# W298/Surtr

Measured on AMD Instinct MI355X. Metric: fragments/sec, higher is better.
Workload: dtype f32

## Files before the change

surtr_amd/csrc/clip_core.h:

```cpp
#pragma once
#include <hip/hip_runtime.h>
#include <stdint.h>
#ifndef SURTR_LANES
#define SURTR_LANES 64
#define SURTR_LSH 6
#endif
#ifndef SURTR_WG
#define SURTR_WG 256
#endif
#if SURTR_LANES == 64
#define SURTR_WG_WIDE (4u * SURTR_WG)
#else
#define SURTR_WG_WIDE SURTR_WG
#endif
#define SURTR_NWAVE_WIDE (SURTR_WG_WIDE / SURTR_LANES)
#define SURTR_NWAVE (SURTR_WG / SURTR_LANES)
#ifndef SURTR_DBG
#define SURTR_DBG(...)
#endif

#ifdef SURTR_STAMP
__device__ unsigned long long g_stamp[96];
__device__ unsigned long long g_stamp2[64];
#ifdef SURTR_STAMP_SMALL
// ... 65 lines not shown
}

struct InLds
{
    typedef uint16_t off_t; typedef uint8_t len_t; typedef uint16_t idx_t;
    static constexpr uint32_t SENT = 0xFFFEu, REM = 0xFFFFu, MAXLEN = 255u;
};
struct InGlobal
{
    typedef uint32_t off_t; typedef uint32_t len_t; typedef uint32_t idx_t;
    static constexpr uint32_t SENT = 0xFFFFFFFEu, REM = 0xFFFFFFFFu, MAXLEN = 0x7FFFFFFFu;
};

template <class TT>
struct Topo
{
    typename TT::off_t* loff; typename TT::len_t* llen; typename TT::idx_t* ring;
    uint8_t* fc;
    int8_t* gcomp;
    float* pos;
    uint32_t* succ; uint32_t* pred; uint32_t* pcnt;
    uint32_t* aux0; uint32_t* aux1; uint32_t* aux2; uint32_t* aux3;
    uint2* blk;
    uint32_t capV, capH;
    uint32_t nS, nLive, hUsed;
    uint32_t kcur, n0cur; bool zmode;

    __device__ __forceinline__ int cmp(uint32_t v) const
    {
        if (zmode) return gcomp[v];
        const uint32_t f = fc[v];
        return f < kcur ? SURTR_DEAD : (f == kcur ? -1 : (v >= n0cur ? 2 : 1));
    }
    __device__ __forceinline__ bool alive(uint32_t v) const { return fc[v] >= kcur; }
    __device__ __forceinline__ void kill(uint32_t v) { fc[v] = (uint8_t)kcur; if (zmode) gcomp[v] = -1; }
};

struct Shared
{
    float4 planes[SURTR_MAXF + 1];
    union {
        float4 pmar[SURTR_MAXF + 1];
        uint32_t pw[4 * (SURTR_MAXF + 1)];
    };
    uint32_t hist[SURTR_MAXF + 1];
    uint32_t zhist[SURTR_MAXF + 1];
    uint32_t nzero[SURTR_MAXF + 1];
    uint32_t wsum[2 * SURTR_NWAVE_WIDE];
    uint32_t flagBad, flagErr;
    uint32_t deg7;
    uint32_t pf[3][8];
    uint32_t changed;
    uint32_t misc[8];
    uint32_t cutmask[4];
#ifdef SURTR_STAMP
    unsigned long long ph[16];
#endif
};

struct SolidIn
{
    const float* pos;
    const uint32_t* loff;
    const uint32_t* llen;
    const int32_t* nbr;
    uint32_t nv;
    const uint8_t* tri;
    const float* rad;
    const uint32_t* perm; const float4* posr_s; const float4* bsph;
};

__device__ __forceinline__ float plane_dist(const float4 pl, float x, float y, float z)
{
    float t = pl.x * x + pl.y * y;
    t = t + pl.z * z;
    return pl.w + t;
}

__device__ __forceinline__ int side_of(float s)
{
    if (fabsf(s) < 1.0e-10f) return 0;
    float m = -s;
    return m > 0.f ? 1 : (m < 0.f ? -1 : 0);
}

__device__ __forceinline__ uint32_t group_size() { return blockDim.x; }
__device__ __forceinline__ uint32_t group_waves() { return blockDim.x >> SURTR_LSH; }

__device__ __forceinline__ uint2 wave_incl_scan2(uint2 v)
{
    v.x += dpp_move<0x111, 0xF>(0u, v.x); v.y += dpp_move<0x111, 0xF>(0u, v.y);
    v.x += dpp_move<0x112, 0xF>(0u, v.x); v.y += dpp_move<0x112, 0xF>(0u, v.y);
    v.x += dpp_move<0x114, 0xF>(0u, v.x); v.y += dpp_move<0x114, 0xF>(0u, v.y);
    v.x += dpp_move<0x118, 0xF>(0u, v.x); v.y += dpp_move<0x118, 0xF>(0u, v.y);
    v.x += dpp_move<0x142, 0xA>(0u, v.x); v.y += dpp_move<0x142, 0xA>(0u, v.y);
    v.x += dpp_move<0x143, 0xC>(0u, v.x); v.y += dpp_move<0x143, 0xC>(0u, v.y);
    return v;
}

__device__ __forceinline__ uint2 wave_excl2(uint2 c)
{
    uint2 s = wave_incl_scan2(c);
    return make_uint2(s.x - c.x, s.y - c.y);
}

__device__ inline void scan_block_array(uint32_t nb, uint2* blk, Shared& sh, uint32_t& totC, uint32_t& totW)
{
    const uint32_t l = lane_id(), w = wave_id();
    uint2 carry = make_uint2(0u, 0u);
    for (uint32_t c0 = 0; c0 < nb; c0 += group_size())
    {
        const uint32_t i = c0 + threadIdx.x;
        uint2 x = make_uint2(0u, 0u);
        if (i < nb) x = blk[i];
        uint2 inc = wave_incl_scan2(x);
        if (l == SURTR_LANES - 1u) { sh.wsum[2 * w] = inc.x; sh.wsum[2 * w + 1] = inc.y; }
        __syncthreads();
        uint2 woff = make_uint2(0u, 0u), tot = make_uint2(0u, 0u);
        for (uint32_t q = 0; q < group_waves(); ++q)
        {
            const uint32_t a = sh.wsum[2 * q], bq = sh.wsum[2 * q + 1];
            if (q < w) { woff.x += a; woff.y += bq; }
            tot.x += a; tot.y += bq;
        }
        if (i < nb) blk[i] = make_uint2(carry.x + woff.x + inc.x - x.x, carry.y + woff.y + inc.y - x.y);
        carry.x += tot.x; carry.y += tot.y;
        __syncthreads();
    }
    totC = carry.x; totW = carry.y;
}

template <class Fn>
__device__ void scan_blocks(uint32_t n, uint2* blk, Shared& sh, Fn fn, uint32_t& totC, uint32_t& totW)
{
    const uint32_t nb = (n + SURTR_LANES - 1u) >> SURTR_LSH;
    const uint32_t l = lane_id(), w = wave_id();
    for (uint32_t b = w; b < nb; b += group_waves())
    {
        const uint32_t i = (b << SURTR_LSH) + l;
        uint2 c = make_uint2(0u, 0u);
        if (i < n) c = fn(i);
        uint2 s = wave_incl_scan2(c);
        if (l == SURTR_LANES - 1u) blk[b] = s;
    }
    __syncthreads();
    scan_block_array(nb, blk, sh, totC, totW);
}

template <class I>
__device__ __forceinline__ uint32_t face_next(const I* ring, uint32_t len, uint32_t prev)
{
    if (len <= 4u)
    {
        const uint32_t l1 = len > 1u ? 1u : 0u, l2 = len > 2u ? 2u : 0u, l3 = len > 3u ? 3u : 0u;
        const uint32_t e0 = ring[0], e1 = ring[l1], e2 = ring[l2], e3 = ring[l3];
        const uint32_t last = len == 4u ? e3 : (len == 3u ? e2 : (len == 2u ? e1 : e0));
        if (e0 == prev) return last;
        if (len > 1u && e1 == prev) return e0;
        if (len > 2u && e2 == prev) return e1;
        if (len > 3u && e3 == prev) return e2;
        return last;
    }
    uint32_t k = 0;
    while (k < len && (uint32_t)ring[k] != prev) ++k;
    if (k == 0) return (uint32_t)ring[len - 1];
    return (uint32_t)ring[k - 1];
// ... 766 lines not shown
        const uint32_t n0 = nS, n1 = nS + M;
        const uint32_t nref = T.nLive + (k ? sh.hist[k - 1u] : dropTotal) + M;
        if ((clist.l || cutcnt.l) && T.hUsed + 3u * M + 8u > wtop)
        {
            for (uint32_t i = tid; i < nC; i += group_size()) { if (clist.l) T.aux3[i] = clist.l[i]; if (cutcnt.l) T.aux2[i] = cutcnt.l[i]; }
            __syncthreads();
            clist.l = nullptr; cutcnt.l = nullptr; wtop = T.capH;
        }
        const uint32_t wfloor = T.hUsed + 3u * M;
        const WArr<uint16_t> srcv = carve16(M, wfloor, T.succ);
        const WArr<uint8_t> srcj = carve8(M, wfloor, T.aux1);
        const WArr<uint16_t> wpred = carve16(M, wfloor, T.pred);
        const WArr<uint16_t> wsave = carve16(M, wfloor, T.aux0);
        {
            bool dup = false;
            uint32_t run = 0;
            for (uint32_t q = 0; q < w; ++q) run += sh.wsum[q];
            for (uint32_t b = cb0; b < cb1; ++b)
            {
                const uint32_t i = (b << SURTR_LSH) + l;
                uint2 c = make_uint2(0u, 0u);
                uint32_t km = 0;
                if (i < nC) { km = cutcnt.get(i); c.x = (km & 0x8000u) ? (km & 0x7FFFu) : (uint32_t)__builtin_popcount(km); }
                const uint2 s2 = wave_incl_scan2(c);
                const uint32_t base = run;
                run += lane_bcast(s2.x, SURTR_LANES - 1u);
                if (i < nC && c.x)
                {
                    const uint32_t v = clist.get(i);
                    uint32_t t = base + s2.x - c.x;
                    if (MULTIWAVE && !(km & 0x8000u))
                    {
                        if (c.x >= 2u)
                        {
                            const I* r2 = T.ring + T.loff[v];
                            for (uint32_t mm = km; mm; mm &= mm - 1u)
                            {
                                const uint32_t ja = (uint32_t)__builtin_ctz(mm), ua = r2[ja];
                                for (uint32_t lo = km & ((1u << ja) - 1u); lo; lo &= lo - 1u) if ((uint32_t)r2[__builtin_ctz(lo)] == ua) dup = true;
                            }
                        }
                        for (uint32_t mm = km; mm; mm &= mm - 1u) { srcv.set(t, v); srcj.set(t, (uint32_t)__builtin_ctz(mm)); ++t; }
                        continue;
                    }
                    const I* r = T.ring + T.loff[v];
                    const uint32_t deg = T.llen[v];
                    for (uint32_t j0 = 0; j0 < deg; j0 += 4)
                    {
                        uint32_t u[4]; int cu[4];
#pragma unroll
                        for (int q = 0; q < 4; ++q) u[q] = r[j0 + q < deg ? j0 + q : deg - 1u];
#pragma unroll
                        for (int q = 0; q < 4; ++q) cu[q] = T.cmp(u[q] < TT::SENT ? u[q] : 0u);
#pragma unroll
                        for (int q = 0; q < 4; ++q)
                        {
                            const uint32_t j = j0 + q;
                            if (j >= deg || u[q] >= TT::SENT || cu[q] <= 0) continue;
                            srcv.set(t, v); srcj.set(t, j); ++t;
                            for (uint32_t jj = 0; jj < j; ++jj) if ((uint32_t)r[jj] == u[q]) dup = true;
                        }
                    }
                }
            }
            if (dup) pf[3] = 1;
            __syncthreads();
            STAMP(9);
            const bool ordered = pf[3] != 0;
            for (uint32_t t = tid; t < M; t += group_size())
            {
                const uint32_t v = srcv.get(t), j = srcj.get(t), fresh = n0 + t;
                I* r = T.ring + T.loff[v];
                const uint32_t u = r[j];
                const float ax = T.pos[3 * v], ay = T.pos[3 * v + 1], az = T.pos[3 * v + 2];
                const float bx = T.pos[3 * u], by = T.pos[3 * u + 1], bz = T.pos[3 * u + 2];
                const float sa = plane_dist(pl, ax, ay, az);
                const float sb = plane_dist(pl, bx, by, bz);
                const float inv = 1.f / (sb - sa);
                T.pos[3 * fresh] = (ax * sb - bx * sa) * inv;
                T.pos[3 * fresh + 1] = (ay * sb - by * sa) * inv;
                T.pos[3 * fresh + 2] = (az * sb - bz * sa) * inv;
                {
                    const float nx = T.pos[3 * fresh], ny = T.pos[3 * fresh + 1], nz = T.pos[3 * fresh + 2];
                    uint32_t f = SURTR_NEVER;
                    for (uint32_t q = k + 1u; q < F; ++q)
                    {
                        const int cq = side_of(plane_dist(sh.planes[q], nx, ny, nz));
                        if (cq < 0) { f = q; break; }
                        if (cq == 0) atomicAdd(&sh.nzero[q], 1u);
                    }
                    T.fc[fresh] = (uint8_t)f;
                    if (T.zmode) T.gcomp[fresh] = 2;
                }
                const uint32_t lo = T.hUsed + 3u * t;
                T.loff[fresh] = (typename TT::off_t)lo; T.llen[fresh] = 2;
                T.ring[lo] = (I)v; T.ring[lo + 1] = (I)u; T.ring[lo + 2] = (I)TT::REM;
                wpred.set(t, 0u);
                if (!ordered)
                {
                    I* ru = T.ring + T.loff[u];
                    const uint32_t du = T.llen[u];
                    for (uint32_t q = 0; q < du; ++q) if ((uint32_t)ru[q] == v) { ru[q] = (I)fresh; break; }
                    r[j] = (I)fresh;
                }
            }
            STAMP(10);
            if (ordered) __syncthreads();
            if (ordered && tid == 0)
            {
                COUNT(39);
                for (uint32_t t = 0; t < M; ++t)
                {
                    const uint32_t v = srcv.get(t), fresh = n0 + t, u = T.ring[T.loff[fresh] + 1u];
                    I* ru = T.ring + T.loff[u];
                    const uint32_t du = T.llen[u];
                    for (uint32_t q = 0; q < du; ++q) if ((uint32_t)ru[q] == v) { ru[q] = (I)fresh; break; }
                    T.ring[T.loff[v] + srcj.get(t)] = (I)fresh;
                }
            }
        }
        uint32_t hend = T.hUsed + 3u * M;
        if (tid == 0) sh.misc[6] = 0;
        __syncthreads();
        STAMP(5);

        bool serial = anyZero;
        if (!serial)
        {
            bool bad = false, longw = false;
            const WArr<uint16_t> wsucc = srcv;
            auto finish = [&](uint32_t t, uint32_t X, uint32_t c) {
                if (c >= TT::SENT || c < n0 || c == X || T.cmp(c) != 2) { bad = true; wsucc.set(t, X); }
                else
                {
                    wsucc.set(t, c);
                    wpred.set(c - n0, X);
                }
            };
            for (uint32_t t = tid; t < M; t += group_size())
            {
                const uint32_t X = n0 + t;
                uint32_t prev = X, c = T.ring[T.loff[X]], steps = 0;
                bool clipped;
                while (true)
                {
                    const uint32_t cc = c < TT::SENT ? c : 0u;
                    const int cm = T.cmp(cc); const uint32_t lo = T.loff[cc], len = T.llen[cc];
                    clipped = c < TT::SENT && cm == -1;
                    if (!clipped || steps >= SURTR_WALK0) break;
                    const uint32_t hold = c;
                    c = face_next(T.ring + lo, len, prev);
                    prev = hold; ++steps;
                }
                if (clipped) { wsave.set(t, prev + 1u); wsucc.set(t, c); longw = true; continue; }
                wsave.set(t, 0u);
                finish(t, X, c);
            }
            if (longw) pf[7] = 1;
            if (bad) pf[4] = 1;
            __syncthreads();
            STAMP(12);
            COUNT(43);
            if (pf[7] != 0)
            {
                COUNT(40);
                const uint32_t jfloor = T.hUsed + 3u * M;
                const WArr<uint16_t> chain = carve16(nC, jfloor, T.aux2);
                const WArr<uint16_t> jump = carve16(n0, jfloor, T.pcnt);
                for (uint32_t i = tid; i < nC; i += group_size())
                {
                    const uint32_t v = clist.get(i);
                    if (T.llen[v] != 3u) continue;
                    const uint32_t p = T.ring[T.loff[v]];
// ... 269 lines not shown
```

surtr_amd/csrc/prep_sorted.h:

```cpp
#pragma once
#include "wave_clip.h"

#define PS_NEVER 0x7Fu
#ifndef SURTR_PS_NB
#define SURTR_PS_NB 896u
#endif
#ifndef SURTR_SPH_FAN
#define SURTR_SPH_FAN 8u
#endif

namespace surtr {

struct SortedRings
{
    const SRow* row_s; const uint32_t* iperm;
    const float4* bsph2; const float4* bsph3;
};

__device__ __forceinline__ uint32_t ps_sphere_fc(const Shared& sh, const uint32_t F, const float4 sp, const uint32_t k0, uint32_t& kstop)
{
    const float mag = fabsf(sp.x) + fabsf(sp.y) + fabsf(sp.z) + sp.w;
    for (uint32_t k = k0; k < F; ++k)
    {
        const float4 mk = sh.pmar[k];
// ... 59 lines not shown
        if (k < F)
        {
            const float4 pk = sh.planes[k];
            const float n1 = fabsf(pk.x) + fabsf(pk.y) + fabsf(pk.z);
            const float n2 = sqrtf(pk.x * pk.x + pk.y * pk.y + pk.z * pk.z) * 1.0001f;
            sh.pmar[k] = make_float4(n2 * 1.00101f, 1.0e-5f * fabsf(pk.w), 1.0e-5f * n1, 0.f);
        }
    }
    if (tid == 0) { sh.flagErr = 0; sh.flagBad = 0; sh.deg7 = 0; for (int q = 0; q < 7; ++q) sh.misc[q] = 0; }
    const uint32_t nbV = (V + SURTR_LANES - 1u) >> SURTR_LSH;
    for (uint32_t q = tid; q < UBW; q += G) ub[q] = 0u;
    __syncthreads();
    const uint32_t nsb = (V + SURTR_SB - 1u) / SURTR_SB;
    const uint32_t nb2 = (nsb + SURTR_SPH_FAN - 1u) / SURTR_SPH_FAN, nb3 = (nb2 + SURTR_SPH_FAN - 1u) / SURTR_SPH_FAN;
    uint32_t* list2 = (uint32_t*)lbuf;
    uint32_t* list3 = list2 + nb2 + 8u;
    auto verts_in = [&](uint32_t g0, uint32_t g1) -> uint32_t {
        const uint32_t a = g0 * SURTR_SB, b = g1 * SURTR_SB;
        return (b < V ? b : V) - (a < V ? a : V);
    };
    for (uint32_t s3 = tid; s3 < nb3; s3 += G)
    {
        uint32_t ks = 0;
        const uint32_t f = ps_sphere_fc(sh, F, sr.bsph3[s3], 0u, ks);
        const uint32_t g0 = s3 * SURTR_SPH_FAN * SURTR_SPH_FAN;
        if (f != 0xFFu) atomicAdd(&sh.hist[f], verts_in(g0, g0 + SURTR_SPH_FAN * SURTR_SPH_FAN));
        else list3[atomicAdd(&sh.misc[1], 1u)] = s3 | (ks << 16);
    }
    __syncthreads();
    const uint32_t nU3 = sh.misc[1];
    for (uint32_t t = tid; t < nU3 * SURTR_SPH_FAN; t += G)
    {
        const uint32_t e3 = list3[t / SURTR_SPH_FAN];
        const uint32_t s2 = (e3 & 0xFFFFu) * SURTR_SPH_FAN + t % SURTR_SPH_FAN;
        if (s2 >= nb2) continue;
        uint32_t ks = 0;
        const uint32_t f = ps_sphere_fc(sh, F, sr.bsph2[s2], e3 >> 16, ks);
        if (f != 0xFFu) atomicAdd(&sh.hist[f], verts_in(s2 * SURTR_SPH_FAN, s2 * SURTR_SPH_FAN + SURTR_SPH_FAN));
        else list2[atomicAdd(&sh.misc[2], 1u)] = s2 | (ks << 16);
    }
    __syncthreads();
    const uint32_t nU2 = sh.misc[2];
    for (uint32_t t = tid; t < nU2 * SURTR_SPH_FAN; t += G)
    {
        const uint32_t e2 = list2[t / SURTR_SPH_FAN];
        const uint32_t sb = (e2 & 0xFFFFu) * SURTR_SPH_FAN + t % SURTR_SPH_FAN;
        if (sb >= nsb) continue;
        uint32_t ks = 0;
        const uint32_t f = ps_sphere_fc(sh, F, in.bsph[sb], e2 >> 16, ks);
        if (f != 0xFFu) atomicAdd(&sh.hist[f], verts_in(sb, sb + 1u));
        else atomicOr(&ub[sb >> 5], 1u << (sb & 31u));
    }
    __syncthreads();
    {
        uint32_t carry = 0;
        for (uint32_t q0 = 0; q0 < UBW; q0 += G)
        {
            const uint32_t q = q0 + tid;
            const uint32_t c = q < UBW ? (uint32_t)__builtin_popcount(ub[q]) : 0u;
            const uint32_t inc = wave_incl_scan2(make_uint2(c, 0u)).x;
            if (l == SURTR_LANES - 1u) sh.wsum[w] = inc;
            __syncthreads();
            uint32_t woff = 0, tot = 0;
            for (uint32_t x = 0; x < nw; ++x) { const uint32_t a = sh.wsum[x]; if (x < w) woff += a; tot += a; }
            if (q < UBW)
            {
                uint32_t at = carry + woff + inc - c;
                pre[q] = at;
                for (uint32_t m = ub[q]; m; m &= m - 1u) und[at++] = (uint16_t)(32u * q + (uint32_t)__builtin_ctz(m));
            }
            carry += tot;
            __syncthreads();
        }
        if (tid == 0) sh.misc[4] = carry;
    }
    __syncthreads();
    const uint32_t nUnd = sh.misc[4];
#ifdef SURTR_STAMP
    if (tid == 0 && V > 10000u) { atomicAdd(&g_stamp[45], (unsigned long long)nUnd); atomicAdd(&g_stamp[46], (unsigned long long)nsb); }
#endif
    STAMP(44);
    constexpr uint32_t GPW = SURTR_LANES / SURTR_SB;
    const uint32_t nWork = (nUnd + GPW - 1u) / GPW;
    for (uint32_t wb = w; wb < nWork; wb += nw)
    {
        const uint32_t sub = wb * GPW + l / SURTR_SB;
        const bool okg = sub < nUnd;
        const uint32_t i = (okg ? (uint32_t)und[sub] : 0u) * SURTR_SB + (l % SURTR_SB);
        const bool valid = okg && i < V;
        const float4 pr = in.posr_s[valid ? i : 0u];
        const float mag = fabsf(pr.x) + fabsf(pr.y) + fabsf(pr.z);
        uint32_t f = PS_NEVER, z = 0u;
        bool done = !valid, clear = true;
        for (uint32_t k = 0; k < F; ++k)
        {
            if (__all(done)) break;
            const float4 mk = sh.pmar[k];
            const float s = plane_dist(sh.planes[k], pr.x, pr.y, pr.z);
            const bool cut = s >= 1.0e-10f, zz = fabsf(s) < 1.0e-10f, live = !done;
            const bool far = fabsf(s) > __builtin_fmaf(pr.w, mk.x, __builtin_fmaf(mk.z, mag, mk.y));
            clear = clear & (far | !live);
            z |= (live & zz) ? 0x80u : 0u;
            f = (live & cut) ? k : f;
            done = done | cut;
        }
        const uint32_t at = sub * SURTR_SB + (l % SURTR_SB);
        if (valid) { if (at < kCap) vfc[at] = (uint8_t)(f | z); else vfc_g[at] = (uint8_t)(f | z); }
        const bool never = valid && f == PS_NEVER;
        const bool drop = valid && !never && clear;
        const bool need = valid && !never && !clear;
        wave_hist_add(sh.hist, f, drop);
        ps_append16(needy, &sh.misc[3], need, i);
        if (__ballot(never))
        {
            const uint32_t v = never ? in.perm[i] : 0u;
            const uint32_t deg = never ? in.llen[v] : 0u;
            if (never && z) sh.misc[5] = 1u;
            ps_append(klist, &sh.misc[6], never, i | ((f | z) << 16) | ((deg < 255u ? deg : 255u) << 24));
        }
    }
    __syncthreads();
    STAMP(0);
    const uint32_t nNeedy = sh.misc[3];
#ifdef SURTR_STAMP
    if (tid == 0 && V > 10000u) atomicAdd(&g_stamp[47], (unsigned long long)nNeedy);
#endif
    for (uint32_t t0 = w << SURTR_LSH; t0 < nNeedy; t0 += G)
    {
        const uint32_t t = t0 + l;
        const bool valid = t < nNeedy;
        const uint32_t i = valid ? (uint32_t)needy[t] : 0u;
        const SRow row = sr.row_s[i];
        uint32_t byte;
        {
            const uint32_t g = i / SURTR_SB, word = ub[g >> 5], bit = g & 31u;
            const uint32_t at = (pre[g >> 5] + (uint32_t)__builtin_popcount(word & ((1u << bit) - 1u))) * SURTR_SB + i % SURTR_SB;
            byte = (valid && at < kCap) ? (uint32_t)vfc[valid ? at : 0u] : 0u;
            if (valid && at >= kCap) byte = vfc_g[at];
        }
        const uint32_t f = byte & 0x7Fu;
        const uint32_t hd = row.w[0] & 0xFFFFu;
        const uint32_t deg = valid ? (hd & 7u) : 0u, notri = (hd >> 7) & 1u, big = (hd >> 6) & 1u;
        uint32_t uq[7], on[7], fq[7];
#pragma unroll
        for (int q = 0; q < 7; ++q)
        {
            const uint32_t x = row.w[(q + 1) >> 1];
            const uint32_t u = (uint32_t)q < deg ? (((q + 1) & 1) ? (x >> 16) : (x & 0xFFFFu)) : 0u;
            const uint32_t g = u / SURTR_SB, word = ub[g >> 5], bit = g & 31u;
            on[q] = ((uint32_t)q < deg ? 1u : 0u) & ((word >> bit) & 1u);
            uq[q] = (pre[g >> 5] + (uint32_t)__builtin_popcount(word & ((1u << bit) - 1u))) * SURTR_SB + u % SURTR_SB;
        }
#pragma unroll
        for (int q = 0; q < 7; ++q) fq[q] = (on[q] && uq[q] < kCap) ? ((uint32_t)vfc[uq[q]] & 0x7Fu) : f;
#pragma unroll
        for (int q = 0; q < 7; ++q) if (on[q] && uq[q] >= kCap) fq[q] = (uint32_t)vfc_g[uq[q]] & 0x7Fu;
        bool differ = false;
#pragma unroll
        for (int q = 0; q < 7; ++q) differ = differ | (fq[q] != f);
        const bool walk = valid && (big != 0u || (notri != 0u && !differ));
        const bool keep = valid && differ && !walk, drop = valid && !differ && !walk;
        if (keep && (byte & 0x80u)) sh.misc[5] = 1u;
        ps_append(klist, &sh.misc[6], keep, i | (byte << 16) | (deg << 24));
        if (__ballot(walk))
        {
            const uint32_t v = walk ? in.perm[i] : 0u;
            ps_append(walks, &sh.misc[0], walk, v | (f << 24));
        }
        wave_hist_add(sh.hist, f, drop);
        if (drop && (byte & 0x80u))
        {
            const float4 pr = in.posr_s[i];
            for (uint32_t k = 0; k < f; ++k)
                if (side_of(plane_dist(sh.planes[k], pr.x, pr.y, pr.z)) == 0) atomicAdd(&sh.zhist[k], 1u);
        }
    }
    __syncthreads();
    if (sh.misc[0] != 0u) prepass_exact<4>(in, F, sh, (unsigned long long*)nullptr, (uint2*)nullptr, walks, sh.misc[0], klist, &sh.misc[6], sr.iperm);
    __syncthreads();
    STAMP(1);
    const uint32_t n = sh.misc[6];
    for (uint32_t b = tid; b < nbV; b += G) { bmask[b] = 0ull; bblk[b] = make_uint2(0u, 0u); }
    __syncthreads();
    for (uint32_t t = tid; t < n; t += G)
    {
        const uint32_t ke = klist[t];
        const uint32_t v = in.perm[ke & 0xFFFFu], deg = ke >> 24;
        atomicOr(&bmask[v >> SURTR_LSH], 1ull << (v & (SURTR_LANES - 1u)));
// ... 222 lines not shown
```

surtr_amd/csrc/wave_clip.h:

```cpp
#pragma once
#include "clip_core.h"

#ifndef SURTR_WR
#define SURTR_WR 3584u
#endif
#ifndef SURTR_WNL
#define SURTR_WNL 2560u
#endif
#ifndef SURTR_WWALK0
#define SURTR_WWALK0 4u
#endif
#define WC_MAXF 64u
#define WC_MAXN 0x2000u
#define WC_BAIL 102
#define WC_SENT 0xFFFEu
#define WC_NONE 0xFFFFu
#define WC_WHY_WORDS 29u
static_assert(CUR_WC_WHY + WC_WHY_WORDS <= CUR_STATS_WORDS, "the why[] block ends inside what surtr_queue_stats copies out");
#define WC_RET(site) do { if (threadIdx.x == 0u) atomicAdd(&why[site], 1u); SURTR_DBG("record clip: pair handed on at site %d\n", site); return WC_BAIL; } while (0)
#ifdef SURTR_STAMP
__device__ unsigned long long g_wstamp[64];
__device__ unsigned long long g_wplane[32];
__device__ uint32_t g_wneed[4 * 8192];
#define WSTAMP_DECL unsigned long long ws_t0 = __builtin_readcyclecounter(), ws_t1
// ... 509 lines not shown
        auto fring = [&](uint32_t at) -> uint32_t { return at >= LT::kNL ? at - LT::kNL : at; };
        auto xof = [&](uint32_t t) -> uint32_t { return WC_MAXN + (t < fromf ? (uint32_t)W.freel[fring(fh0 + t)] : tbase + (t - fromf)); };
        for (uint32_t q = tid; q < bmw; q += G) wc_st32(B, bm + 2u * q, 0u);
        WSTAMP(3);
        WCOUNT(18, 1); WCOUNT(19, nC); WCOUNT(20, M); WCOUNT(21, nl);
#ifdef SURTR_STAMP
        if (tid == 0u) { const unsigned long long need = 2ull * (4u * rtop + (8u * LT::kNR - ltop)); if (need > W.ph[31]) W.ph[31] = need; if (k >= 2u && need > W.ph[29]) W.ph[29] = need; }
#endif
        auto kfn2 = [&](uint32_t i, uint32_t& aux) -> uint2 {
            const uint32_t id = clipped_id(i), km = wc_ld8(B, ckm8 + i);
            if (!(km & 0x80u)) { aux = id << 8; return make_uint2(0u, 0u); }
            aux = km | (id << 8) | (((tail_ld(id) >> 8) & 7u) << 24);
            return make_uint2(1u, (uint32_t)__builtin_popcount(km & 0x7Fu));
        };
        wc_rr_place<2>(W, sc, NI, st2, kfn2, [&](uint32_t i, uint32_t xc, uint32_t xm, uint2 c, uint32_t aux) {
            const uint32_t km = aux & 0x7Fu, id = (aux >> 8) & 0xFFFFu, len = aux >> 24;
            if (!c.x) { nout[i - xc] = (uint16_t)id; return; }
            wc_st16(B, cbase + i, xm);
            tail_st(id, 0x8000u | (len << 12) | i);
            if (i >= nCo) { W.freel[fring(fpush + (xc - nCo))] = (uint16_t)(id - WC_MAXN); wc_st16(B, clist + (xc - nCo), i); }
            uint32_t t = xm;
            for (uint32_t m = km; m; m &= m - 1u, ++t) { wc_st16(B, src + t, i | ((uint32_t)__builtin_ctz(m) << 12)); wc_st16(B, srcid + t, id); }
        });
        cur ^= 1u;
        WSTAMP(15);
        __syncthreads();
        WSTAMP(4);
        const uint32_t nref = nLive + (k ? SURTR_UNIFORM(W.hist[k - 1u]) : dropTotal) + M;
        bool fail = false;
        auto walk = [&](uint32_t& cv, uint32_t& pcv, uint32_t& p, WcRec& rc, uint32_t& steps, const uint32_t limit, const bool jump) -> uint32_t {
            while (true)
            {
                if (jump && p == 0u && pcv >= nCo)
                {
                    const uint32_t a = wc_ld32(B, nd + 2u * (pcv - nCo)), jx = a & 0xFFFFu;
                    if (jx != pcv) { pcv = jx; cv = clipped_id(jx); steps += a >> 16; rc = rec_of(cv); }
                }
                const uint32_t kmc = wc_ld8(B, ckm8 + pcv);
                if ((kmc >> p) & 1u) return wc_ld16(B, cbase + pcv) + (uint32_t)__builtin_popcount(kmc & ((1u << p) - 1u));
                if (steps >= limit) return WC_NONE;
                const uint32_t e = rc.e(p);
                if (((e >= WC_SENT ? 1u : 0u) | ((e < WC_MAXN ? 1u : 0u) & ((e < b0 ? 1u : 0u) | (e >= b1 ? 1u : 0u))) | (steps + 2u >= nref ? 1u : 0u)) != 0u)
                { SURTR_DBG("  wc walk: sentinel / not clipped / bound e=%u steps=%u nref=%u k=%u\n", e, steps, nref, k); fail = true; return WC_NONE; }
                ++steps;
                const WcRec re = rec_of(e);
                const uint32_t te = re.tail();
                if (!(te & 0x8000u)) { SURTR_DBG("  wc walk: vertex %u not clipped now (tail %x) k=%u\n", e, te, k); fail = true; return WC_NONE; }
                const uint32_t le = (te >> 12) & 7u, q = re.find(cv, le);
                if (q >= le) { SURTR_DBG("  wc walk: no way back k=%u\n", k); fail = true; return WC_NONE; }
                p = q ? q - 1u : le - 1u; cv = e; pcv = te & 0xFFFu; rc = re;
            }
        };
        auto arrive = [&](uint32_t t, uint32_t end) {
            wc_st16(B, wst + t, 0xFFFFu);
            uint32_t* word = (uint32_t*)(void*)(B + 2u * (size_t)(bm + 2u * (end >> 5)));
            const uint32_t before = atomicOr(word, 1u << (end & 31u));
            if (((end == t ? 1u : 0u) | ((before >> (end & 31u)) & 1u)) != 0u) { SURTR_DBG("  wc walk: ends on itself / second arrival t=%u end=%u k=%u\n", t, end, k); fail = true; }
            const uint32_t X = xof(t), Z = xof(end);
            wc_st16(B, 4u * (Z - WC_MAXN), X);
            wc_st16(B, 4u * (X - WC_MAXN) + 1u, Z);
        };
        bool paused = false;
        uint32_t myz0 = 0, myz1 = 0;
        uint16_t* nnow = W.nlist[cur];
        for (uint32_t t = tid; t < M; t += G)
        {
            const uint32_t s = wc_ld16(B, src + t);
            const uint32_t v = wc_ld16(B, srcid + t), j = s >> 12;
            uint32_t pcv = s & 0xFFFu, cv = v;
            WcRec rc = rec_of(cv);
            const uint32_t u = rc.e(j);
            const float4 pa = *(v < WC_MAXN ? g.gpos + v : g.cpos + (v - WC_MAXN));
            const float4 pb = *(u < WC_MAXN ? g.gpos + u : g.cpos + (u - WC_MAXN));
            WcW4 wru = WcW4{0u, 0u, 0u, 0u};
            if (u < WC_MAXN) wru = g.grec[u];
            const uint32_t lv = (rc.tail() >> 12) & 7u;
            uint32_t p = j ? j - 1u : lv - 1u, steps = 0;
            const uint32_t end = walk(cv, pcv, p, rc, steps, walk0, false);
            const uint32_t X = xof(t), ux = X - WC_MAXN;
            const float sa = plane_dist(pl, pa.x, pa.y, pa.z), sb = plane_dist(pl, pb.x, pb.y, pb.z);
            const float inv = 1.f / (sb - sa);
            const float nx = (pa.x * sb - pb.x * sa) * inv, ny = (pa.y * sb - pb.y * sa) * inv, nz = (pa.z * sb - pb.z * sa) * inv;
            g.cpos[ux] = make_float4(nx, ny, nz, 0.f);
            uint32_t f = SURTR_NEVER;
            for (uint32_t q = k + 1u; q < F; ++q)
            {
                const int cq = side_of(plane_dist(W.planes[q], nx, ny, nz));
                if (cq < 0) { f = q; break; }
                if (cq == 0) { if (q < 32u) myz0 |= 1u << q; else myz1 |= 1u << (q - 32u); }
            }
            wc_st32(B, 4u * ux + 2u, u | ((f | (3u << 8)) << 16));
            nnow[keepn + t] = (uint16_t)X;
            const WcRec ru = u < WC_MAXN ? WcRec{wru.a, wru.b, wru.c, wru.d} : wc_rec(B, 8u * (u - WC_MAXN), true);
            const uint32_t tu = ru.tail(), qu = ru.find(v, (tu >> 8) & 7u);
            if ((tu & 0x8000u) || qu >= ((tu >> 8) & 7u)) { SURTR_DBG("  wc patch: kept end does not link the clipped vertex k=%u\n", k); fail = true; }
            else if (u < WC_MAXN) { const uint16_t xv = (uint16_t)X; __builtin_memcpy(GB + 16u * (size_t)u + 2u * qu, &xv, 2); }
            else wc_st16(B, 4u * (u - WC_MAXN) + qu, X);
            if (end != WC_NONE) arrive(t, end);
            else { wc_st16(B, wst + t, pcv | (p << 12)); paused = true; }
        }
        const bool anyPaused = wc_any(W, ac, paused, 0u);
        WSTAMP(5);
        if (anyPaused)
        {
            WCOUNT(24, 1);
            for (uint32_t ci = tid; ci < nCn; ci += G)
            {
                const uint32_t i = wc_ld16(B, clist + ci);
                const uint32_t c = clipped_id(i);
                const WcRec r = rec_of(c);
                const uint32_t e0 = r.e(0u);
                uint32_t nx = i, d = 0;
                if (!(wc_ld8(B, ckm8 + i) & 1u) && e0 >= WC_MAXN && e0 < WC_SENT)
                {
                    const WcRec r0 = rec_of(e0);
                    const uint32_t t0 = r0.tail();
                    if ((t0 & 0x8000u) && r0.find(c, (t0 >> 12) & 7u) == 1u) { nx = t0 & 0xFFFu; d = 1u; }
                }
                wc_st32(B, nd + 2u * (i - nCo), nx | (d << 16));
            }
            __syncthreads();
            for (uint32_t round = 0; round < 12u; ++round)
            {
                bool ch = false;
                for (uint32_t ci = tid; ci < nCn; ci += G)
                {
                    const uint32_t i = wc_ld16(B, clist + ci);
                    const uint32_t a = wc_ld32(B, nd + 2u * (i - nCo)), j1 = a & 0xFFFFu;
                    if (j1 == i) continue;
                    const uint32_t b2 = wc_ld32(B, nd + 2u * (j1 - nCo)), j2 = b2 & 0xFFFFu;
                    if (j2 == j1) continue;
                    const uint32_t b3 = wc_ld32(B, nd + 2u * (j2 - nCo)), j3 = b3 & 0xFFFFu;
                    wc_st32(B, nd + 2u * (i - nCo), j3 | (((a >> 16) + (b2 >> 16) + (j3 != j2 ? (b3 >> 16) : 0u)) << 16));
                    ch = true;
                }
                if (!wc_any(W, ac, ch, 0u)) break;
            }
            WSTAMP(6);
            for (uint32_t t = tid; t < M; t += G)
            {
                const uint32_t ws = wc_ld16(B, wst + t);
                if (ws == 0xFFFFu) continue;
                uint32_t pcv = ws & 0xFFFu, cv = clipped_id(pcv), p = ws >> 12, steps = walk0;
                WcRec rc = rec_of(cv);
                const uint32_t end = walk(cv, pcv, p, rc, steps, 0xFFFFFFFFu, true);
                if (end != WC_NONE) arrive(t, end);
                else fail = true;
#ifdef SURTR_STAMP
                atomicAdd(&g_wstamp[22], (unsigned long long)steps); atomicMax(&g_wstamp[23], (unsigned long long)steps);
#endif
            }
            WSTAMP(7);
        }
        if (myz0) atomicOr(&W.zm[0], myz0);
        if (myz1) atomicOr(&W.zm[1], myz1);
        if (wc_any(W, ac, fail || bad, 1u)) WC_RET(11);
        WSTAMP(8);
        zmask |= (unsigned long long)SURTR_UNIFORM(W.zm[0]) | ((unsigned long long)SURTR_UNIFORM(W.zm[1]) << 32);
        nLive = nLive - nC + M; nl = keepn + M;
        WSTAMP(9);
#ifdef SURTR_STAMP
        if (tid == 0u) { int c = 0; while (c < 7 && (32u << c) < NI) ++c; atomicAdd(&g_wplane[2 * c], 1ull); atomicAdd(&g_wplane[2 * c + 1], __builtin_readcyclecounter() - pl_t0); }
#endif
        if (nLive + dropAlive < 4u) { nLive = 0; break; }
    }
    __syncthreads();
    out.nl = nl; out.nLive = nLive; out.rtop = rtop; out.cur = cur;
    ctr.ac = ac; ctr.sc = sc;
    return 0;
}

template <class LT, class AR, class PR>
__device__ __attribute__((always_inline)) inline int wc_park(LT& W, const uint32_t F, const uint32_t n, const WcOut o, const WcGlob g,
// ... 105 lines not shown
```

Baseline: 1.210 million.

## Chunk plane tests and software-pipeline vertex loads in classification loops

Replaces the per-plane early-exit loops that find the first cutting plane with a chunked version. It loads C planes at once, evaluates them branch-free, and checks for wave-wide completion only once per chunk; the zero-distance bookkeeping is redone afterward in a separate pass. The prep loop now prefetches the next iteration's vertex index and position one iteration ahead to hide global load latency. The trade-off is wasted plane evaluations past the first cut and a second pass over planes when zero-distance hits occur.

```diff
diff --git a/surtr_amd/csrc/clip_core.h b/surtr_amd/csrc/clip_core.h
--- a/surtr_amd/csrc/clip_core.h
+++ b/surtr_amd/csrc/clip_core.h
@@ -171,6 +171,71 @@
     if (fabsf(s) < 1.0e-10f) return 0;
     float m = -s;
     return m > 0.f ? 1 : (m < 0.f ? -1 : 0);
+}
+
+#ifndef SURTR_PLANE_CHUNK
+#define SURTR_PLANE_CHUNK 4u
+#endif
+#ifndef SURTR_PLANE_CHUNK_GEN
+#define SURTR_PLANE_CHUNK_GEN 2u
+#endif
+#ifndef SURTR_PLANE_CHUNK_P1
+#define SURTR_PLANE_CHUNK_P1 2u
+#endif
+#define SURTR_PLANE_NONE 0x100u
+
+__device__ __forceinline__ uint32_t umin32(uint32_t a, uint32_t b) { return a < b ? a : b; }
+
+template <uint32_t C, class ZF>
+__device__ __forceinline__ uint32_t planes_first_cut(const float4* planes, const uint32_t q0, const uint32_t F, const float x, const float y, const float z, ZF&& on_zero)
+{
+    uint32_t f = SURTR_NEVER, zf = SURTR_NEVER;
+    for (uint32_t k0 = q0; k0 < F; k0 += C)
+    {
+        float4 pl[C];
+#pragma unroll
+        for (uint32_t c = 0; c < C; ++c) pl[c] = planes[umin32(k0 + c, F - 1u)];
+        uint32_t fc = SURTR_PLANE_NONE, zc = SURTR_PLANE_NONE;
+#pragma unroll
+        for (uint32_t c = C; c-- > 0u;)
+        {
+            const float s = plane_dist(pl[c], x, y, z);
+            fc = s >= 1.0e-10f ? c : fc;
+            zc = !(fabsf(s) >= 1.0e-10f) ? c : zc;
+        }
+        f = umin32(f, k0 + fc); zf = umin32(zf, k0 + zc);
+        if (__all(f != SURTR_NEVER)) break;
+    }
+    if (zf < f)
+        for (uint32_t q = zf; q < F && q < f; ++q)
+            if (side_of(plane_dist(planes[q], x, y, z)) == 0) on_zero(q);
+    return f;
+}
+
+template <uint32_t C, uint32_t NEVER>
+__device__ __forceinline__ void planes_first_cut_ball(const float4* planes, const float4* pmar, const uint32_t F, const float x, const float y, const float z,
+                                                      const float rad, const float mag, const bool active, uint32_t& f_out, bool& inplane_out, bool& clear_out)
+{
+    uint32_t f = NEVER, zf = NEVER, nf = NEVER;
+    for (uint32_t k0 = 0; k0 < F; k0 += C)
+    {
+        float4 pl[C], mk[C];
+#pragma unroll
+        for (uint32_t c = 0; c < C; ++c) { const uint32_t k = umin32(k0 + c, F - 1u); pl[c] = planes[k]; mk[c] = pmar[k]; }
+        uint32_t fc = SURTR_PLANE_NONE, zc = SURTR_PLANE_NONE, nc = SURTR_PLANE_NONE;
+#pragma unroll
+        for (uint32_t c = C; c-- > 0u;)
+        {
+            const float s = plane_dist(pl[c], x, y, z);
+            const float margin = __builtin_fmaf(rad, mk[c].x, __builtin_fmaf(mk[c].z, mag, mk[c].y));
+            fc = s >= 1.0e-10f ? c : fc;
+            zc = fabsf(s) < 1.0e-10f ? c : zc;
+            nc = fabsf(s) > margin ? nc : c;
+        }
+        f = umin32(f, k0 + fc); zf = umin32(zf, k0 + zc); nf = umin32(nf, k0 + nc);
+        if (__all(!active | (f != NEVER))) break;
+    }
+    f_out = f; inplane_out = zf < f; clear_out = (nf > f) | (nf == NEVER);
 }
 
 __device__ __forceinline__ uint32_t group_size() { return blockDim.x; }
@@ -1103,13 +1168,7 @@
                 T.pos[3 * fresh + 2] = (az * sb - bz * sa) * inv;
                 {
                     const float nx = T.pos[3 * fresh], ny = T.pos[3 * fresh + 1], nz = T.pos[3 * fresh + 2];
-                    uint32_t f = SURTR_NEVER;
-                    for (uint32_t q = k + 1u; q < F; ++q)
-                    {
-                        const int cq = side_of(plane_dist(sh.planes[q], nx, ny, nz));
-                        if (cq < 0) { f = q; break; }
-                        if (cq == 0) atomicAdd(&sh.nzero[q], 1u);
-                    }
+                    const uint32_t f = planes_first_cut<SURTR_PLANE_CHUNK_GEN>(sh.planes, k + 1u, F, nx, ny, nz, [&](uint32_t q) { atomicAdd(&sh.nzero[q], 1u); });
                     T.fc[fresh] = (uint8_t)f;
                     if (T.zmode) T.gcomp[fresh] = 2;
                 }
diff --git a/surtr_amd/csrc/prep_sorted.h b/surtr_amd/csrc/prep_sorted.h
--- a/surtr_amd/csrc/prep_sorted.h
+++ b/surtr_amd/csrc/prep_sorted.h
@@ -165,28 +165,31 @@
     STAMP(44);
     constexpr uint32_t GPW = SURTR_LANES / SURTR_SB;
     const uint32_t nWork = (nUnd + GPW - 1u) / GPW;
-    for (uint32_t wb = w; wb < nWork; wb += nw)
-    {
+    auto und_at = [&](uint32_t wb) -> uint32_t {
         const uint32_t sub = wb * GPW + l / SURTR_SB;
-        const bool okg = sub < nUnd;
-        const uint32_t i = (okg ? (uint32_t)und[sub] : 0u) * SURTR_SB + (l % SURTR_SB);
-        const bool valid = okg && i < V;
-        const float4 pr = in.posr_s[valid ? i : 0u];
+        return sub < nUnd ? (uint32_t)und[sub] : 0xFFFFFFFFu;
+    };
+    auto vert_of = [&](uint32_t g) -> uint32_t {
+        const uint32_t i = g * SURTR_SB + (l % SURTR_SB);
+        return (g != 0xFFFFFFFFu && i < V) ? i : 0xFFFFFFFFu;
+    };
+    const uint32_t wu = SURTR_UNIFORM(w);
+    uint32_t i_nx = vert_of(und_at(wu));
+    uint32_t g_nx2 = und_at(wu + nw);
+    float4 pr_nx = in.posr_s[i_nx != 0xFFFFFFFFu ? i_nx : 0u];
+    for (uint32_t wb = wu; wb < nWork; wb += nw)
+    {
+        const uint32_t sub = wb * GPW + l / SURTR_SB;
+        const uint32_t i = i_nx;
+        const bool valid = i != 0xFFFFFFFFu;
+        const float4 pr = pr_nx;
+        i_nx = vert_of(g_nx2);
+        g_nx2 = und_at(wb + 2u * nw);
+        pr_nx = in.posr_s[i_nx != 0xFFFFFFFFu ? i_nx : 0u];
         const float mag = fabsf(pr.x) + fabsf(pr.y) + fabsf(pr.z);
-        uint32_t f = PS_NEVER, z = 0u;
-        bool done = !valid, clear = true;
-        for (uint32_t k = 0; k < F; ++k)
-        {
-            if (__all(done)) break;
-            const float4 mk = sh.pmar[k];
-            const float s = plane_dist(sh.planes[k], pr.x, pr.y, pr.z);
-            const bool cut = s >= 1.0e-10f, zz = fabsf(s) < 1.0e-10f, live = !done;
-            const bool far = fabsf(s) > __builtin_fmaf(pr.w, mk.x, __builtin_fmaf(mk.z, mag, mk.y));
-            clear = clear & (far | !live);
-            z |= (live & zz) ? 0x80u : 0u;
-            f = (live & cut) ? k : f;
-            done = done | cut;
-        }
+        uint32_t f; bool inpl, clear;
+        planes_first_cut_ball<SURTR_PLANE_CHUNK_P1, PS_NEVER>(sh.planes, sh.pmar, F, pr.x, pr.y, pr.z, pr.w, mag, valid, f, inpl, clear);
+        const uint32_t z = inpl ? 0x80u : 0u;
         const uint32_t at = sub * SURTR_SB + (l % SURTR_SB);
         if (valid) { if (at < kCap) vfc[at] = (uint8_t)(f | z); else vfc_g[at] = (uint8_t)(f | z); }
         const bool never = valid && f == PS_NEVER;
diff --git a/surtr_amd/csrc/wave_clip.h b/surtr_amd/csrc/wave_clip.h
--- a/surtr_amd/csrc/wave_clip.h
+++ b/surtr_amd/csrc/wave_clip.h
@@ -615,13 +615,8 @@
             const float inv = 1.f / (sb - sa);
             const float nx = (pa.x * sb - pb.x * sa) * inv, ny = (pa.y * sb - pb.y * sa) * inv, nz = (pa.z * sb - pb.z * sa) * inv;
             g.cpos[ux] = make_float4(nx, ny, nz, 0.f);
-            uint32_t f = SURTR_NEVER;
-            for (uint32_t q = k + 1u; q < F; ++q)
-            {
-                const int cq = side_of(plane_dist(W.planes[q], nx, ny, nz));
-                if (cq < 0) { f = q; break; }
-                if (cq == 0) { if (q < 32u) myz0 |= 1u << q; else myz1 |= 1u << (q - 32u); }
-            }
+            const uint32_t f = planes_first_cut<SURTR_PLANE_CHUNK>(W.planes, k + 1u, F, nx, ny, nz,
+                                                                   [&](uint32_t q) { if (q < 32u) myz0 |= 1u << q; else myz1 |= 1u << (q - 32u); });
             wc_st32(B, 4u * ux + 2u, u | ((f | (3u << 8)) << 16));
             nnow[keepn + t] = (uint16_t)X;
             const WcRec ru = u < WC_MAXN ? WcRec{wru.a, wru.b, wru.c, wru.d} : wc_rec(B, 8u * (u - WC_MAXN), true);
```

New measurement: 1.255 million (median of 6 runs). 1.04x the previous value.
